# MP-Gadget/shenqi

Measured on AMD Instinct MI355X. Metric: particle-steps/sec (grav+PM+SPH) at 256^3; rms force error vs ref, higher is better.
Workload: dtype f64

## Files before the change

### include/shenqi_hip.h

```cpp
#ifndef SHENQI_HIP_H
#define SHENQI_HIP_H

#include <stddef.h>
#include <stdint.h>

#ifdef __cplusplus
extern "C" {
#endif

#define SHQ_OK 0
#define SHQ_ERR_INVALID 1
#define SHQ_ERR_DEVICE 2
#define SHQ_ERR_NOMEM 3
#define SHQ_ERR_STATE 4
#define SHQ_ERR_NOCONV 5

#define SHQ_NGRAVTAB 512
#define SHQ_NMAXCHILD 8
#define SHQ_NODELISTLENGTH 4
#define SHQ_TIMEBINS 46

typedef struct shq_context shq_context;


// ... 350 lines not shown
    double Imom[3][3];
    double Jmom[3];
    double MaxDens;
    int64_t first_member;
} shq_fof_group;
int shq_fof(shq_context *ctx, const shq_fof_params *params, const uint64_t *ids, uint64_t *minid_by_particle, int32_t *grnr_by_particle,
            int64_t *ngroups);
int shq_fof_groups_download(shq_context *ctx, shq_fof_group *groups, int64_t capacity);
int shq_fof_group_sums(shq_context *ctx, const double *values_by_particle, int ncol, double *sums_by_group);
int shq_fof_seed_select(shq_context *ctx, double MinFoFMassForNewSeed, double MinMStarForNewSeed, int32_t *d_seed_index, int64_t capacity, int64_t *nseeds);
int shq_fof_members(shq_context *ctx, int32_t *members, int64_t capacity, int64_t *nmembers);

typedef struct shq_bh_dyn_view {
    void *base;
    size_t elsize;
    int64_t numslots;
    size_t off_mintimebin, off_timebindynfric, off_jumptominpot;
    size_t off_dfaccel, off_df_surroundingvel, off_dragaccel;
    size_t off_minpotpos, off_minpotvel;
} shq_bh_dyn_view;
int shq_bh_dynamics_upload(shq_context *ctx, const shq_part_view *parts, const shq_bh_dyn_view *bh);
int shq_bh_dynamics_download(shq_context *ctx, const shq_part_view *parts, const shq_bh_dyn_view *bh);
int shq_set_bh_reposition(shq_context *ctx, int enabled);
int shq_kick_bh(shq_context *ctx, const double gravkick[SHQ_TIMEBINS + 1], const int32_t *active, int64_t nactive);
int shq_grav_short_run(shq_context *ctx, const shq_grav_params *params, const int32_t *active,
                       int64_t nactive, int update_potential, int walk_mode);
int shq_grav_short_run_range(shq_context *ctx, const shq_grav_params *params, int64_t first, int64_t count,
                             int update_potential, int walk_mode);
int shq_set_walk_stats(shq_context *ctx, int level);
int shq_set_walk_launch(shq_context *ctx, int persist, int leaf_ring);
int shq_set_walk_sparse(shq_context *ctx, int enable);
int shq_walk_pair_lean(shq_context *ctx);
int shq_set_walk_overlap(shq_context *ctx, int mode);
int shq_walk_pair_status(shq_context *ctx, int64_t *recovered_launches, int64_t *stack_high_water, int64_t *last_mopped_tasks);
int shq_set_walk_debug(shq_context *ctx, int pair_spin_max, int pair_stack_cap);
int shq_set_tree_debug(shq_context *ctx, int64_t initial_node_cap);
int shq_tree_build_attempts(shq_context *ctx, int *attempts);
int shq_direct_force_sample(shq_context *ctx, const double *sample_pos, int64_t ns, int64_t nsrc, double BoxSize, double G, double h,
                            int repeat, double *accel);
int shq_grav_short_download(shq_context *ctx, double (*accel)[3], double *potential,
                            int64_t *ninteractions, shq_walk_stats *stats);
typedef struct shq_grav_query {
    double Pos[3];
    int32_t NodeList[4];
    double OldAcc;
} shq_grav_query;
typedef struct shq_grav_result {
    double Acc[3];
    double Potential;
} shq_grav_result;
int shq_grav_short_secondary(shq_context *ctx, const shq_grav_params *params, const shq_grav_query *queries, int64_t nq,
                             shq_grav_result *results, int64_t *ninteractions, int update_potential);
typedef struct shq_data_index {
    int32_t Task;
    int32_t Index;
    int32_t NodeList[4];
} shq_data_index;
int shq_toptree_upload(shq_context *ctx, const shq_tree_view *tree, const shq_topleaf *topleaves, int ntopleaves);
int shq_grav_toptree_exports(shq_context *ctx, const shq_grav_params *params, const int32_t *active, int64_t nactive,
                             int32_t *exportcounts, shq_data_index *table, int64_t capacity, int64_t *nexport);
int shq_ngb_toptree_exports(shq_context *ctx, int symmetric, double BoxSize, const int32_t *active, int64_t nactive,
                            int32_t *exportcounts, shq_data_index *table, int64_t capacity, int64_t *nexport);
int shq_grav_toptree_exports_resident(shq_context *ctx, const shq_grav_params *params, const int32_t *active, int64_t nactive,
                                      int active_on_device, int ntask, int64_t *nexport, int64_t *task_counts);
int shq_grav_export_pack(shq_context *ctx, shq_grav_query *d_queries, int32_t *d_place);
int shq_grav_reduce_export_results(shq_context *ctx, const int32_t *place, const shq_grav_result *results, int64_t n,
// ... 904 lines not shown
```

### shenqi_amd/capi.py

```python
import ctypes as C
import os

import numpy as np

_HERE = os.path.dirname(os.path.abspath(__file__))
LIBDIR = os.environ.get("SHQ_LIBDIR") or os.path.join(_HERE, "lib")
DATADIR = os.path.join(_HERE, "data")

NGRAVTAB = 512
NMAXCHILD = 8
NOFIELD = C.c_size_t(-1).value

WALK_EXACT = 0
WALK_GROUP = 1
WALK_AUTO = 2
WALK_TREE_ORDER = 0x100
WALK_DEFER_POSTPROCESS = 0x200


class ShqError(RuntimeError):
    """Non-zero status from the library (the shim's endrun() equivalent)."""


def _load(name):
# ... 378 lines not shown
TOPLEAF_DTYPE = np.dtype([("Task", "<i4"), ("topnode", "<i4"), ("treenode", "<i4")])
DATA_INDEX_DTYPE = np.dtype([("Task", "<i4"), ("Index", "<i4"), ("NodeList", "<i4", 4)])
hip.shq_grav_reduce_export_results.argtypes = [_vp, _vp, _vp, C.c_int64, C.c_int]
hip.shq_grav_reduce_export_results.restype = C.c_int
hip.shq_grav_postprocess.argtypes = [_vp, C.POINTER(GravParams), _vp, C.c_int64, C.c_int]
hip.shq_grav_postprocess.restype = C.c_int
hip.shq_toptree_upload.argtypes = [_vp, C.POINTER(TreeView), _vp, C.c_int]
hip.shq_toptree_upload.restype = C.c_int
hip.shq_grav_toptree_exports.argtypes = [_vp, C.POINTER(GravParams), _vp, C.c_int64, _vp, _vp, C.c_int64, C.POINTER(C.c_int64)]
hip.shq_grav_toptree_exports.restype = C.c_int
hip.shq_ngb_toptree_exports.argtypes = [_vp, C.c_int, C.c_double, _vp, C.c_int64, _vp, _vp, C.c_int64, C.POINTER(C.c_int64)]
hip.shq_ngb_toptree_exports.restype = C.c_int
hip.shq_grav_toptree_exports_resident.argtypes = [_vp, C.POINTER(GravParams), _vp, C.c_int64, C.c_int, C.c_int, C.POINTER(C.c_int64), _vp]
hip.shq_grav_toptree_exports_resident.restype = C.c_int
hip.shq_grav_export_pack.argtypes = [_vp, _vp, _vp]
hip.shq_grav_export_pack.restype = C.c_int
GAS_NCOL = 28
hip.shq_gas_set_device.argtypes = [_vp, _vp, C.c_int64, C.c_int64]
hip.shq_gas_get_device.argtypes = [_vp, _vp, C.c_int64, C.c_int]
hip.shq_density_resident.argtypes = [_vp, C.POINTER(DensityParams), C.POINTER(SphStats)]
hip.shq_hydro_resident.argtypes = [_vp, C.POINTER(HydroParams), C.POINTER(SphStats)]
for _f in ("shq_gas_set_device", "shq_gas_get_device", "shq_density_resident", "shq_hydro_resident"):
    getattr(hip, _f).restype = C.c_int
hip.shq_set_walk_stats.argtypes = [_vp, C.c_int]
hip.shq_set_walk_stats.restype = C.c_int
hip.shq_set_walk_launch.argtypes = [_vp, C.c_int, C.c_int]
hip.shq_set_walk_launch.restype = C.c_int
hip.shq_set_walk_sparse.argtypes = [_vp, C.c_int]
hip.shq_set_walk_sparse.restype = C.c_int
hip.shq_walk_pair_lean.argtypes = [_vp]
hip.shq_walk_pair_lean.restype = C.c_int
hip.shq_set_walk_overlap.argtypes = [_vp, C.c_int]
hip.shq_set_walk_overlap.restype = C.c_int
hip.shq_pm_set_fft_transposed.argtypes = [_vp, C.c_int]
hip.shq_pm_set_fft_transposed.restype = C.c_int
hip.shq_walk_pair_status.argtypes = [_vp, C.POINTER(C.c_int64), C.POINTER(C.c_int64), C.POINTER(C.c_int64)]
hip.shq_walk_pair_status.restype = C.c_int
hip.shq_set_walk_debug.argtypes = [_vp, C.c_int, C.c_int]
hip.shq_set_walk_debug.restype = C.c_int
hip.shq_set_tree_debug.argtypes = [_vp, C.c_int64]
hip.shq_set_tree_debug.restype = C.c_int
hip.shq_tree_build_attempts.argtypes = [_vp, C.POINTER(C.c_int)]
hip.shq_tree_build_attempts.restype = C.c_int
hip.shq_direct_force_sample.argtypes = [_vp, _vp, C.c_int64, C.c_int64, C.c_double, C.c_double, C.c_double, C.c_int, _vp]
hip.shq_direct_force_sample.restype = C.c_int
hip.shq_exchange_plan.argtypes = [_vp, C.POINTER(ExchangeLayout), _vp, C.c_int64, _vp, C.c_int, C.c_int, C.c_int64, C.POINTER(C.c_int64), C.POINTER(C.c_int64), _vp]
hip.shq_exchange_pack.argtypes = [_vp, C.POINTER(ExchangeLayout), _vp, _vp, C.c_int64, _vp, C.c_int, _vp, _vp]
hip.shq_exchange_unpack.argtypes = [_vp, C.POINTER(ExchangeLayout), _vp, C.c_int64, _vp, _vp, _vp, C.c_int]
hip.shq_slots_gc.argtypes = [_vp, C.POINTER(ExchangeLayout), _vp, C.POINTER(C.c_int64), C.c_int64, _vp, _vp, _vp]
hip.shq_slots_gc_sorted.argtypes = [_vp, C.POINTER(ExchangeLayout), _vp, C.POINTER(C.c_int64), C.c_int64, _vp, _vp, _vp]
hip.shq_slots_split_particles.argtypes = [_vp, C.POINTER(ExchangeLayout), C.POINTER(SpawnLayout), _vp, C.POINTER(C.c_int64), C.c_int64, _vp, _vp, C.c_int64, _vp]
hip.shq_slots_convert.argtypes = [_vp, C.POINTER(ExchangeLayout), _vp, C.c_int64, C.c_int64, _vp, _vp, _vp, _vp, C.c_int64, C.c_int]
hip.shq_make_particle_stars.argtypes = [_vp, C.POINTER(ExchangeLayout), C.POINTER(StarSpawnLayout), _vp, C.c_int64, C.c_int64, _vp, _vp, _vp, _vp, _vp, C.c_int64, C.c_double]
hip.shq_blackhole_make_seeds.argtypes = [_vp, C.POINTER(ExchangeLayout), C.POINTER(BhSeedLayout), _vp, C.c_int64, C.c_int64, _vp, _vp, _vp, _vp, _vp, C.c_int64,
                                         C.c_double, C.c_double]
hip.shq_bh_accretion.argtypes = [_vp, C.POINTER(TreeView), C.POINTER(PartView), C.POINTER(SphView), C.POINTER(BhSlotView), _vp, _vp, C.c_int64, C.POINTER(KickFactors),
                                 C.POINTER(BhParams), C.c_int64, _vp, C.c_int64, C.POINTER(BhWork)]
hip.shq_bh_feedback.argtypes = [_vp, C.POINTER(TreeView), C.POINTER(PartView), C.POINTER(SphView), C.POINTER(BhSlotView), _vp, _vp, C.c_int64, C.POINTER(KickFactors),
                                C.POINTER(BhParams), C.c_int64, _vp, C.c_int64, _vp, C.POINTER(BhWork), C.POINTER(C.c_int64), C.POINTER(C.c_int64)]
hip.shq_bh_accretion.restype = hip.shq_bh_feedback.restype = C.c_int
hip.shq_winds_and_feedback.argtypes = [_vp, C.POINTER(TreeView), C.POINTER(PartView), C.POINTER(SphView), C.POINTER(StarView), _vp, _vp, C.c_int64, C.POINTER(WindParams),
                                       _vp, C.c_int64, _vp, _vp, C.c_int64, C.POINTER(C.c_int64), C.POINTER(C.c_int64)]
hip.shq_winds_and_feedback.restype = C.c_int
hip.shq_winds_candidates.argtypes = [_vp, C.POINTER(TreeView), C.POINTER(PartView), C.POINTER(SphView), C.POINTER(StarView), _vp, _vp, C.c_int64, C.POINTER(WindParams),
                                     _vp, C.c_int64, _vp, _vp, C.c_int64, C.POINTER(C.c_int64)]
hip.shq_winds_apply.argtypes = [_vp, C.POINTER(PartView), C.POINTER(SphView), _vp, _vp, C.c_int64, C.POINTER(WindParams), _vp, C.c_int64, C.POINTER(C.c_int64)]
# ... 862 lines not shown
```

### shenqi_amd/csrc/capi.hip

```cpp
#include "common.hpp"
#include <stdarg.h>
#include <string.h>
#include <stdlib.h>
#include <math.h>
#include <thread>
#include <atomic>
#include <algorithm>

static thread_local char g_err[1024] = "";

void shq_set_error(const char *fmt, ...)
{
    va_list ap;
    va_start(ap, fmt);
    vsnprintf(g_err, sizeof(g_err), fmt, ap);
    va_end(ap);
}

extern "C" const char *shq_last_error(void) { return g_err; }
extern "C" const char *shq_version(void) { return "shenqi_hip 0.1 (gfx950)"; }

namespace {

template <typename F> void parallel_for(int64_t n, F f)
// ... 124 lines not shown
       hipEventCreateWithFlags(&ctx->ev_pair_join, hipEventDisableTiming) != hipSuccess) {
        shq_set_error("creating the pair kernel's stream failed");
        delete ctx;
        return SHQ_ERR_DEVICE;
    }
    if(const char *v = getenv("SHQ_WALK_FREE_CUS")) {
        const int k = atoi(v);
        if(k > 0 && k <= 16) {
            uint32_t mask_walk[8];
            for(int w = 0; w < 8; w++)
                mask_walk[w] = ~0u;
            for(int a = 0; a < 8; a++)
                for(int c = 0; c < k; c++) {
                    const int bit = 32 * a + ((a + c / 4) % 8) + 8 * (c % 4);
                    mask_walk[bit >> 5] &= ~(1u << (bit & 31));
                }
            if(hipExtStreamCreateWithCUMask(&ctx->stream_walk, 8, mask_walk) != hipSuccess ||
               hipEventCreateWithFlags(&ctx->ev_walk_in, hipEventDisableTiming) != hipSuccess ||
               hipEventCreateWithFlags(&ctx->ev_walk_out, hipEventDisableTiming) != hipSuccess) {
                shq_set_error("creating the CU-masked walk stream failed");
                delete ctx;
                return SHQ_ERR_DEVICE;
            }
        }
    }
    if(const char *v = getenv("SHQ_PM_OVERLAP"))
        ctx->pm_overlap = atoi(v) != 0;
    if(const char *v = getenv("SHQ_PM_SCRUB"))
        ctx->pm_scrub = atoi(v) != 0;
    if(const char *v = getenv("SHQ_WALK_SPARSE"))
        ctx->walk_sparse = atoi(v);
    if(const char *v = getenv("SHQ_WALK_OVERLAP"))
        ctx->walk_overlap = atoi(v);
    if(const char *v = getenv("SHQ_TREE_TARGETS_REFRESH"))
        ctx->tree_targets_refresh = atoi(v) > 0 ? atoi(v) : 1;
    if(const char *v = getenv("SHQ_FFT_TRANSPOSED"))
        ctx->fft_transposed = atoi(v) != 0;
    if(const char *v = getenv("SHQ_TREEPM_FUSE"))
        ctx->treepm_fuse = atoi(v) != 0;
    if(const char *v = getenv("SHQ_WALK_VARIANT"))
        ctx->walk_variant = atoi(v);
    if(const char *v = getenv("SHQ_WALK_STATS_GUARD"))
        ctx->stats_guard = atoi(v);
    if(const char *v = getenv("SHQ_WALK_PADDING"))
        ctx->allow_padding = atoi(v) != 0;
    if(const char *v = getenv("SHQ_WALK_STATS"))
        ctx->walk_stats = atoi(v);
    if(const char *v = getenv("SHQ_XCD_K"))
        ctx->xcd_k = atoi(v);
    if(const char *v = getenv("SHQ_WALK_PERSIST"))
        ctx->walk_persist = atoi(v);
    if(const char *v = getenv("SHQ_WALK_RING"))
        ctx->walk_ring = atoi(v);
    {
        int ncu = 0;
        if(hipDeviceGetAttribute(&ncu, hipDeviceAttributeMultiprocessorCount, device) == hipSuccess && ncu > 0)
            ctx->num_cus = ncu;
    }
    *out = ctx;
    return SHQ_OK;
}

extern "C" void shq_shutdown(shq_context *ctx)
{
    if(!ctx)
        return;
// ... 65 lines not shown
        (void) hipStreamDestroy(ctx->stream);
    if(ctx->stream_walk)
        (void) hipStreamDestroy(ctx->stream_walk);
    if(ctx->stream_pm)
        (void) hipStreamDestroy(ctx->stream_pm);
    if(ctx->stream_pair)
        (void) hipStreamDestroy(ctx->stream_pair);
    if(ctx->ev_pair_fork)
        (void) hipEventDestroy(ctx->ev_pair_fork);
    if(ctx->ev_pair_join)
        (void) hipEventDestroy(ctx->ev_pair_join);
    for(int i = 0; i < 4; i++)
        if(ctx->ev_sph[i])
            (void) hipEventDestroy(ctx->ev_sph[i]);
    if(ctx->ev_pm_ready)
        (void) hipEventDestroy(ctx->ev_pm_ready);
    if(ctx->ev_pm_done)
        (void) hipEventDestroy(ctx->ev_pm_done);
    delete ctx;
}

extern "C" int shq_set_walk_sparse(shq_context *ctx, int enable)
{
    SHQ_CHECK(ctx, SHQ_ERR_INVALID, "null context");
    ctx->walk_sparse = enable == 2 ? 2 : enable != 0;
    return SHQ_OK;
}

extern "C" int shq_set_walk_overlap(shq_context *ctx, int mode)
{
    SHQ_CHECK(ctx, SHQ_ERR_INVALID, "null context");
    SHQ_CHECK(mode >= 0 && mode <= 2, SHQ_ERR_INVALID, "walk overlap mode %d", mode);
    ctx->walk_overlap = mode;
    return SHQ_OK;
}

extern "C" int shq_walk_pair_lean(shq_context *ctx)
{
    SHQ_CHECK(ctx, SHQ_ERR_INVALID, "null context");
    if(!ctx->node_lean_checked || !ctx->node_lean_bad.ptr)
        return 0;
    SHQ_HIP(hipSetDevice(ctx->device));
    int bad = 1;
    SHQ_HIP(hipMemcpyAsync(&bad, ctx->node_lean_bad.ptr, sizeof(int), hipMemcpyDeviceToHost, ctx->stream));
    SHQ_HIP(hipStreamSynchronize(ctx->stream));
    return bad == 0 ? 1 : 0;
}

extern "C" int shq_set_walk_launch(shq_context *ctx, int persist, int leaf_ring)
{
    SHQ_CHECK(ctx && persist >= 0 && persist <= 2 && (leaf_ring == 0 || leaf_ring == 1), SHQ_ERR_INVALID, "walk launch: persist 0..2, leaf_ring 0 or 1");
    ctx->walk_persist = persist;
    ctx->walk_ring = leaf_ring;
    return SHQ_OK;
}

extern "C" int shq_set_walk_stats(shq_context *ctx, int level)
{
    SHQ_CHECK(ctx && level >= 0 && level <= 2, SHQ_ERR_INVALID, "walk stats level must be 0, 1 or 2");
    ctx->walk_stats = level;
    return SHQ_OK;
}

int shq_join_pm(shq_context *ctx)
{
    if(ctx->pm_pending) {
// ... 1172 lines not shown
```

### shenqi_amd/csrc/common.hpp

```cpp
#ifndef SHQ_COMMON_HPP
#define SHQ_COMMON_HPP

#include <hip/hip_runtime.h>
#include <hipfft/hipfft.h>
#include <stdint.h>
#include <stdio.h>
#include <string>
#include <vector>
#include "../../include/shenqi_hip.h"
#include "yields_math.hpp"
#include "cooling_math.hpp"

void shq_set_error(const char *fmt, ...);

#define SHQ_HIP(call)                                                                          \
    do {                                                                                       \
        hipError_t e_ = (call);                                                                \
        if(e_ != hipSuccess) {                                                                 \
            shq_set_error("%s:%d: %s failed: %s", __FILE__, __LINE__, #call, hipGetErrorString(e_)); \
            return (e_ == hipErrorOutOfMemory) ? SHQ_ERR_NOMEM : SHQ_ERR_DEVICE;               \
        }                                                                                      \
    } while(0)

#define SHQ_CHECK(cond, code, ...)                                                             \
// ... 389 lines not shown
    bool pm_measure_power = false;
    bool have_power = false;
    int ps_nbins = 0, ps_bintab_n = 0;
    DevBuf<double> ps_sums;
    DevBuf<int32_t> ps_bintab;
    bool pm_spec_pending = false;
    shq_pm_params pm_spec_params = {};
    int pm_spec_route = 0;
    DevBuf<double> pm_fac;
    bool pm_fac_set = false;
    DevBuf<double> pm_fac_one;
    int pm_typemask = -1;
    DevBuf<double> slab_fac;
    bool ps_slab = false;
    bool have_types = false;

    shq_walk_stats last_stats = {};
    int walk_variant = 3;
    int walk_stats = 0;
    int walk_persist = 1;
    int walk_ring = 1;
    int num_cus = 256;
    DevBuf<unsigned int> walk_tasks;
    DevBuf<int4> sp_items, sp_stack;
    DevBuf<int32_t> sp_count;
    DevBuf<int> sp_flags;
    PinBuf<int> sp_host;
    int sp_stack_cap = 0;
    unsigned sp_spin_max = 0;
    int walk_sparse = 1;
    DevBuf<int> node_lean_bad;
    bool node_lean_checked = false;
    int walk_overlap = 1;
    bool sp_check_pending = false;
    int xcd_k = 32;
    float last_walk_ms = 0;
    int last_walk_mode = 0;

    PinBuf<char> stage;

    bool uvbg_keep = false;
    int uvbg_n = 0;
    std::vector<float> uvbg_j21, uvbg_xhi;
    double uvbg_ms[4] = {0, 0, 0, 0};
    shq_heiii_stats heiii_stats = {};
    double lens_ms[4] = {0, 0, 0, 0};
    DevBuf<double> zel_spec;
    bool zel_have = false;
    int zel_n = 0, zel_seed = 0, zel_unitary = 0, zel_invert = 0;
    int64_t zel_chunk = 0;
    double zel_ms[4] = {0, 0, 0, 0};
    double glass_ms[4] = {0, 0, 0, 0};
    double thermal_ms[3] = {0, 0, 0};
    bool yld_have = false;
    YieldDesc yld_desc = {};
    std::vector<double> yld_host;
    DevBuf<double> yld_tab, yld_time;
    int64_t yld_time_n = 0;
    double yld_loga0 = 0, yld_dloga = 0, yld_amin = 0, yld_amax = 0;
    DevBuf<double> yld_in, yld_out;
    DevBuf<int32_t> yld_i32;
    DevBuf<uint8_t> yld_mark;
    double yld_ms[2] = {0, 0};
    bool cool_have = false;
    CoolPar cool_par = {};
    double cool_fbar = 0;
// ... 242 lines not shown
```

### shenqi_amd/csrc/grav_walk.hip

```cpp
#include "common.hpp"
#include "pm_readout.hpp"
#include <utility>
#include <stdlib.h>

namespace {

struct WalkArgs {
    const NodeG *nodeG;
    const double4 *posm;
    const double4 *posm_leaf;
    const double *oldacc;
    const int32_t *targets;
    const int32_t *qstart;
    double *acc;
    double *pot;
    int32_t *nint;
    GravStatsDev *stats;
    long long ntargets;
    int root;
    double Box, invBox, halfBox;
    double rcut, rcut2;
    double h, h2, h_inv, h3_inv;
    double inv_celldx;
    double errtol, bh2;
// ... 144 lines not shown
#define SHQ_SPARSE_LANES 8
#endif
#ifndef SHQ_SPARSE_CAP
#define SHQ_SPARSE_CAP 96
#endif
#define SHQ_SPARSE_STACK 4096
#define SHQ_SPARSE_SPIN (1u << 22)
#ifndef SHQ_PAIR_DEPTH2
#define SHQ_PAIR_DEPTH2 1
#endif
enum SpFlag {
    SP_OVERFLOW = 0,
    SP_GAVEUP = 1,
    SP_MOPPED = 2,
    SP_HIGHWATER = 3,
    SP_STICKY_ERROR = 8,
    SP_STICKY_RECOVERED = 9,
    SP_STICKY_HIGHWATER = 10,
    SP_TASK_COUNTER = 16
};
#define SP_TASK_DONE (-2)
#ifndef SHQ_PAIR_WAVES
#define SHQ_PAIR_WAVES 8
#define SHQ_PAIR_WG_PER_CU 2
#define SHQ_PAIR_EU 4
#endif

template <bool POT>
__device__ __forceinline__ void leaf_ring_drain(const double4 *__restrict__ tab, const double4 *ring, unsigned &mymask, double px, double py,
                                                double pz, const WalkArgs &a, double &ax, double &ay, double &az, double &pot,
                                                const unsigned long long wrapm)
{
    asm volatile("s_waitcnt vmcnt(0)" ::: "memory");
    while(shq_ballot(mymask != 0u) != 0ull) {
        if(mymask != 0u) {
            const int b = __builtin_ctz(mymask);
            mymask &= mymask - 1u;
            const double4 q = ring[b];
            leaf_particle<POT>(tab, q, px, py, pz, a, ax, ay, az, pot, wrapm);
        }
    }
}

template <bool POT, bool PREFETCH, int LEAFB, int STATS, bool BH, bool GHOSTS = false, bool PERSIST = false, bool RING = false, bool READOUT = false,
          bool SPARSE = false>
__global__ __launch_bounds__(512) __attribute__((amdgpu_num_sgpr(96), amdgpu_num_vgpr(64))) void grav_walk_exact_kernel(const WalkArgs a)
{
    extern __shared__ double4 ring_all[];
    double4 *const ring = ring_all + (threadIdx.x >> 6) * SHQ_LEAF_RING;
    __shared__ double4 tab[SHQ_NGRAVTAB];
    for(int i = threadIdx.x; i < SHQ_NGRAVTAB; i += blockDim.x) {
        const int j = (i + 1 < SHQ_NGRAVTAB) ? i + 1 : i;
        const double f0 = a.tab_f[i], f1 = a.tab_f[j], p0 = a.tab_p[i], p1 = a.tab_p[j];
        tab[i] = i + 1 < SHQ_NGRAVTAB ? make_double4(f0, f1 - f0, p0, p1 - p0) : make_double4(0, 0, 0, 0);
    }
    __syncthreads();

    typedef const SHQ_CONSTANT_AS NodeG *NodeGK;
    typedef const SHQ_CONSTANT_AS double4 *Double4K;
    const NodeGK nodeG = (NodeGK) (size_t) a.nodeG;
    const Double4K posm_leaf = (Double4K) (size_t) a.posm_leaf;
    const int lane = threadIdx.x & 63;
    int region = blockIdx.x & 7, tried = 0;
    long long wave = PERSIST ? (long long) walk_next_task(walk_cold_args(), region, tried)
                             : (long long) xcd_block(blockIdx.x, gridDim.x, a.xcdK) * (blockDim.x >> 6) + (threadIdx.x >> 6);
    while(wave >= 0) {
    const long long t = wave * 64 + lane;
    long long pi = 0;
    double px = 0, py = 0, pz = 0, aold = 0;
    bool valid;
    {
        const WalkArgs c = PERSIST ? *walk_cold_args() : a;
        valid = t < c.ntargets;
        if(valid) {
            pi = c.targets ? (long long) c.targets[t] : t;
            valid = pi >= 0;
        }
        if(valid) {
// ... 32 lines not shown
                if(u0 + k < c.scrub_n16) {
                    unsigned z = 0;
                    asm volatile("" : "+v"(z));
                    c.scrub[u0 + k] = make_uint4(z, z, z, z);
                }
        }
    }
    double ax = 0, ay = 0, az = 0, pot = 0;
    int nint = 0;
    int sp_n = 0;
    unsigned ringmask = 0;
    int ringfill = 0;
    unsigned long long ringwrap = 0;
    unsigned int node_int_wave = 0;
    int mynext = valid ? a.root : -2;
    int cur = a.root;
    int wrapnode = -1;
    int seg1 = -1, seg2 = -1, seg3 = -1, myend = -1;
    if(GHOSTS) {
        mynext = -2;
        if(valid) {
            const int4 st = *reinterpret_cast<const int4 *>(a.qstart + 4 * t);
            mynext = st.x >= 0 ? st.x : -2;
            seg1 = st.y; seg2 = st.z; seg3 = st.w;
            if(mynext >= 0)
                myend = a.nodeG[mynext].sibling;
        }
    }
    unsigned int visited = 0, wave_applies = 0, wave_node_applies = 0;
    unsigned int hv[8] = {}, hn[8] = {}, hl[8] = {};
    unsigned int lonely8 = 0, lonely16 = 0;

    do {
        NodeG nd = nodeG[cur];
        int wl_hi = __double2hiint(nd.wraplim);
        asm volatile("" : "+s"(wl_hi));
        nd.wraplim = __hiloint2double(wl_hi, __double2loint(nd.wraplim));
        if(STATS)
            visited++;
        const bool act = (mynext == cur);
        if(STATS == 2)
            hv[(__popcll(shq_ballot(mynext == cur)) - 1) >> 3 & 7]++;

        double dx = nd.cofm[0] - px, dy = nd.cofm[1] - py, dz = nd.cofm[2] - pz;
        double ux = nd.center[0] - px, uy = nd.center[1] - py, uz = nd.center[2] - pz;
        double cmax = fmax(fmax(fabs(ux), fabs(uy)), fabs(uz));
        const unsigned long long actm = shq_ballot(mynext == cur);
        if(wl_hi >= 0) {
            asm volatile("" ::: "memory");
            const unsigned long long wrapm = shq_ballot(cmax >= nd.wraplim) & actm;
            if(wrapm != 0ull) {
                wrapnode = cur;
                dx = wrapd(dx, a.Box, a.invBox);
                dy = wrapd(dy, a.Box, a.invBox);
                dz = wrapd(dz, a.Box, a.invBox);
                ux = wrapd(ux, a.Box, a.invBox);
                uy = wrapd(uy, a.Box, a.invBox);
                uz = wrapd(uz, a.Box, a.invBox);
                cmax = fmax(fmax(fabs(ux), fabs(uy)), fabs(uz));
            }
        }
        const double r2 = fma(dz, dz, fma(dy, dy, dx * dx));
        const unsigned long long keepm = actm & ~(shq_ballot(r2 > nd.rcut2) & shq_ballot(cmax > nd.rcuthl));
        const unsigned long long openm = (BH ? 0ull : shq_ballot(nd.mlen2 > r2 * r2 * aold)) | shq_ballot(r2 < nd.bhlim) |
                                         shq_ballot(cmax < nd.inside);
        const unsigned long long acceptm = keepm & ~openm, doopenm = keepm & openm;
        const bool accept = __builtin_amdgcn_inverse_ballot_w64(acceptm), doopen = __builtin_amdgcn_inverse_ballot_w64(doopenm);

        {
            if(STATS && acceptm != 0ull) {
                wave_applies++;
                wave_node_applies++;
                node_int_wave += (unsigned int) __popcll(acceptm);
            }
            if(STATS == 2 && acceptm != 0ull) {
                const int pc = __popcll(acceptm);
                hn[(pc - 1) >> 3 & 7]++;
                if(accept && pc <= 8)
                    lonely8++;
                if(accept && pc <= 16)
                    lonely16++;
            }
            if(accept) {
                apply_accn<POT, false>(tab, dx, dy, dz, r2, nd.mass, a, ax, ay, az, pot);
                nint++;
            }
        }
        if(nd.type == SHQ_PARTICLE_NODE_TYPE) {
            asm volatile("" ::: "memory");
            if(RING && doopenm != 0ull) {
                const int cnt = nd.count;
                if(ringfill + cnt > SHQ_LEAF_RING) {
                    leaf_ring_drain<POT>(tab, ring, ringmask, px, py, pz, a, ax, ay, az, pot, ringwrap);
                    ringfill = 0;
                    ringwrap = 0;
                }
                if(lane < 2 * cnt)
                    __builtin_amdgcn_global_load_lds(reinterpret_cast<const double2 *>(a.posm_leaf + nd.child) + lane,
                                                     (__attribute__((address_space(3))) void *) (ring + ringfill), 16, 0, 0);
                if(doopen) {
                    ringmask |= ((1u << cnt) - 1u) << ringfill;
                    nint += cnt;
                }
                ringfill += cnt;
                if(wrapnode == cur)
                    ringwrap = 1ull;
            }
            if(!RING && doopenm != 0ull) {
                const unsigned long long wrapm = wrapnode == cur ? 1ull : 0ull;
                const Double4K lp = posm_leaf + nd.child;
                const int cnt = nd.count;
                if(STATS)
                    wave_applies += cnt;
                if(STATS == 2) {
                    const int pc = __popcll(doopenm);
                    hl[(pc - 1) >> 3 & 7] += cnt;
                    if(doopen && pc <= 8)
                        lonely8 += cnt;
                    if(doopen && pc <= 16)
                        lonely16 += cnt;
                }
#pragma unroll
                for(int b = 0; b < SHQ_NMAXCHILD; b += LEAFB) {
                    if(b < cnt) {
                        double4 q[LEAFB];
#pragma unroll
                        for(int k = 0; k < LEAFB; k++)
                            q[k] = lp[b + k];
                        if(doopen) {
#pragma unroll
                            for(int k = 0; k < LEAFB; k++)
                                if(b + k < cnt)
                                    leaf_particle<POT>(tab, q[k], px, py, pz, a, ax, ay, az, pot, wrapm);
                        }
                    }
                }
                if(doopen)
                    nint += cnt;
            }
            }
        unsigned long long downm = 0ull;
        int next = nd.sibling;
        if(nd.type == SHQ_NODE_NODE_TYPE) {
            asm volatile("" ::: "memory");
            if(doopenm != 0ull) {
                asm volatile("" ::: "memory");
                downm = doopenm;
                next = nd.child;
                if(SPARSE) {
                    int pc;
                    asm("s_bcnt1_i32_b64 %[pc], %[m]" : [pc] "=s"(pc) : [m] "s"(doopenm) : "scc");
                    if(((pc - (SHQ_SPARSE_LANES + 1)) & (sp_n - SHQ_SPARSE_CAP)) < 0) {
                        if(lane == 0) {
                            unsigned long long *const it = reinterpret_cast<unsigned long long *>(walk_cold_args()->sp_items + (wave * SHQ_SPARSE_CAP + sp_n));
                            agent_store(it, ((unsigned long long) (unsigned) nd.sibling << 32) | (unsigned) nd.child);
                            agent_store(it + 1, doopenm);
                        }
                        sp_n++;
                        downm = 0ull;
                        next = nd.sibling;
                    }
                }
            }
            if(GHOSTS) {
                if(shq_ballot(mynext > cur && (nd.sibling < 0 || mynext < nd.sibling)) != 0ull)
                    next = nd.child;
            }
        }
        {
            const unsigned long long staym = actm & ~downm;
            asm volatile("s_mov_b64 exec, %[m1]\n\t"
                         "v_mov_b32 %[dst], %[sib]\n\t"
                         "s_mov_b64 exec, %[m2]\n\t"
                         "v_mov_b32 %[dst], %[chd]\n\t"
                         "s_mov_b64 exec, -1"
                         : [dst] "+v"(mynext)
                         : [m1] "s"(staym), [m2] "s"(downm), [sib] "s"(nd.sibling), [chd] "s"(nd.child));
        }
        if(GHOSTS && act && mynext == myend) {
            mynext = seg1 >= 0 ? seg1 : -2;
            seg1 = seg2;
            seg2 = seg3;
            seg3 = -1;
            myend = mynext >= 0 ? a.nodeG[mynext].sibling : -1;
        }
        cur = __builtin_amdgcn_readfirstlane(next);
    } while(cur >= 0);

    if(RING)
        leaf_ring_drain<POT>(tab, ring, ringmask, px, py, pz, a, ax, ay, az, pot, ringwrap);
    {
    const WalkArgs c = PERSIST ? *walk_cold_args() : a;
    if(valid) {
        if(SPARSE) {
            agent_store(&c.acc[3 * pi + 0], ax);
            agent_store(&c.acc[3 * pi + 1], ay);
            agent_store(&c.acc[3 * pi + 2], az);
            if(POT)
                agent_store(&c.pot[pi], pot);
            agent_store(&c.nint[pi], (int32_t) nint);
        } else {
            c.acc[3 * pi + 0] = ax;
            c.acc[3 * pi + 1] = ay;
            c.acc[3 * pi + 2] = az;
            if(POT)
                c.pot[pi] = pot;
            c.nint[pi] = nint;
        }
    }
    if(SPARSE) {
        asm volatile("s_waitcnt vmcnt(0)" ::: "memory");
        if(lane == 0)
            agent_store(&c.sp_count[wave], (int32_t) sp_n);
    }
    long long mn = valid ? (long long) nint : __double_as_longlong(sconst(__longlong_as_double(0x7fffffffffffll))), mx = valid ? nint : 0, sm = valid ? nint : 0;
    for(int off = 32; off > 0; off >>= 1) {
        long long o1 = __shfl_xor(mn, off), o2 = __shfl_xor(mx, off), o3 = __shfl_xor(sm, off);
        mn = o1 < mn ? o1 : mn;
        mx = o2 > mx ? o2 : mx;
        sm += o3;
    }
    unsigned int l8s = lonely8, l8m = lonely8, l16s = lonely16, l16m = lonely16;
    if(STATS == 2)
// ... 391 lines not shown
        double M = Box;
        for(int k = 0; k < 3; k++)
            M = fmin(M, fmin(g[i].center[k] - hl, Box - (g[i].center[k] + hl)));
        const double wl = fmax(0.5 * Box - hl, 0.0);
        g[i].wraplim = (len > 0 && wl > 0 && M >= rcut + 1.5 * len) ? -wl : wl;
        if(lean_bad && i < n - 1) {
            const double rootlen = Box * 1.001;
            const int k = lean_level(rootlen, len);
            const LeanProducts lp = lean_products(g[i].mass, len, rcut, Box);
            const bool ok = len > 0 && k >= 0 && k < 32 && ldexp(rootlen, -k) == len && lp.rcuthl == g[i].rcuthl &&
                            lp.mlen2 == g[i].mlen2 && lp.inside == g[i].inside && lp.wraplim == wl;
            if(!ok)
                *lean_bad = 1;
        }
    }
}

__global__ void stats_init_kernel(GravStatsDev *s)
{
    s->ninteractions = 0;
    s->nvisited = 0;
    s->nwave_applies = 0;
    s->nwave_node_applies = 0;
    s->nnode_interactions = 0;
    s->min_int = 0x7fffffffffffll;
    s->max_int = 0;
    for(int b = 0; b < 8; b++)
        s->hist_visit[b] = s->hist_node[b] = s->hist_leaf[b] = 0;
    for(int b = 0; b < 4; b++)
        s->lonely[b] = 0;
}

template <bool POT, bool PREFETCH, int LEAFB, bool BH>
void launch_variant_bh(int stats, bool persist, dim3 grid, dim3 block, hipStream_t stream, const WalkArgs &a, size_t dyn_lds = 0)
{
    constexpr bool RO = !PREFETCH && LEAFB == 2 && !BH;
    if(a.pm_mesh && a.sp_items && RO && !stats && persist && block.x == 512)
        grav_walk_exact_kernel<POT, PREFETCH, LEAFB, 0, BH, false, RO, RO, RO, RO><<<grid, block, dyn_lds, stream>>>(a);
    else if(a.sp_items && RO && !stats && persist && block.x == 512)
        grav_walk_exact_kernel<POT, PREFETCH, LEAFB, 0, BH, false, RO, RO, false, RO><<<grid, block, dyn_lds, stream>>>(a);
    else if(a.pm_mesh && RO && !stats && persist && block.x == 512)
        grav_walk_exact_kernel<POT, PREFETCH, LEAFB, 0, BH, false, RO, RO, RO><<<grid, block, dyn_lds, stream>>>(a);
    else if(a.pm_mesh && RO && !stats && !persist)
        grav_walk_exact_kernel<POT, PREFETCH, LEAFB, 0, BH, false, false, false, RO><<<grid, block, 0, stream>>>(a);
    else if(stats == 2 && POT && !PREFETCH && LEAFB == 2)
        grav_walk_exact_kernel<POT, PREFETCH, LEAFB, (POT && !PREFETCH && LEAFB == 2) ? 2 : 1, BH><<<grid, block, 0, stream>>>(a);
    else if(stats)
        grav_walk_exact_kernel<POT, PREFETCH, LEAFB, 1, BH><<<grid, block, 0, stream>>>(a);
    else if(persist && !PREFETCH && LEAFB == 2 && block.x == 512)
        grav_walk_exact_kernel<POT, PREFETCH, LEAFB, 0, BH, false, (!PREFETCH && LEAFB == 2), (!PREFETCH && LEAFB == 2)><<<grid, block, dyn_lds, stream>>>(a);
    else if(persist && !PREFETCH && LEAFB == 2)
        grav_walk_exact_kernel<POT, PREFETCH, LEAFB, 0, BH, false, (!PREFETCH && LEAFB == 2)><<<grid, block, dyn_lds, stream>>>(a);
    else
        grav_walk_exact_kernel<POT, PREFETCH, LEAFB, 0, BH><<<grid, block, 0, stream>>>(a);
}

template <bool POT, bool PREFETCH, int LEAFB>
void launch_variant(int stats, bool persist, dim3 grid, dim3 block, hipStream_t stream, const WalkArgs &a, size_t dyn_lds = 0)
{
    if(a.useBH)
        launch_variant_bh<POT, PREFETCH, LEAFB, true>(stats, persist, grid, block, stream, a, dyn_lds);
    else
        launch_variant_bh<POT, PREFETCH, LEAFB, false>(stats, persist, grid, block, stream, a, dyn_lds);
}

}

void shq_launch_stats_init(shq_context *ctx) { stats_init_kernel<<<1, 1, 0, ctx->stream>>>(ctx->gstats.ptr); }

void shq_fill_node_walk_params(shq_context *ctx, const shq_grav_params *p)
{
    if((ctx->node_rcut != p->Rcut || ctx->node_bh2 != p->BHOpeningAngle2) && ctx->numnodes > 0) {
        const long long n = ctx->numnodes + 1;
        int *lean_bad = nullptr;
        if(ctx->node_lean_bad.reserve(16) == SHQ_OK && hipMemsetAsync(ctx->node_lean_bad.ptr, 0, sizeof(int) * 16, ctx->stream) == hipSuccess)
            lean_bad = ctx->node_lean_bad.ptr;
        ctx->node_lean_checked = lean_bad != nullptr;
        fill_rcuthl_kernel<<<dim3((unsigned) ((n + 255) / 256)), dim3(256), 0, ctx->stream>>>(ctx->nodeG.ptr, n, p->Rcut, p->BHOpeningAngle2, p->BoxSize, lean_bad);
        ctx->node_rcut = p->Rcut;
        ctx->node_bh2 = p->BHOpeningAngle2;
    }
}

static void fill_walk_args(shq_context *ctx, const shq_grav_params *p, WalkArgs &a)
{
    shq_fill_node_walk_params(ctx, p);
    a.nodeG = ctx->nodeG.ptr;
    a.posm = ctx->posm.ptr;
    a.posm_leaf = ctx->posm_leaf.ptr;
    a.oldacc = ctx->oldacc.ptr;
    a.targets = nullptr;
    a.qstart = nullptr;
    a.acc = ctx->acc.ptr;
    a.pot = ctx->pot.ptr;
    a.nint = ctx->nint.ptr;
    a.stats = ctx->gstats.ptr;
    a.ntargets = 0;
    a.root = ctx->root;
    a.Box = p->BoxSize;
// ... 268 lines not shown
        if(ctx->mesh_words % 2 == 0 && per <= 4096) {
            a.scrub = (uint4 *) ctx->mesh.ptr;
            a.scrub_n16 = n16;
            a.scrub_per_task = (int) per;
            scrubbed = true;
        }
    }
    if(ctx->fuse_readout) {
        SHQ_CHECK(shq_walk_can_fuse_readout(ctx, p, d_active, ntargets, first), SHQ_ERR_STATE, "fused readout requested for a launch that cannot carry it");
        a.pm_mesh = ctx->mesh.ptr;
        a.pmN = ctx->pm_nmesh;
        a.pmzp = ctx->pm_zp;
        a.pmcell = ctx->fuse_cell;
        a.pmffac = ctx->fuse_ffac;
        a.G = ctx->fuse_G;
        a.treeacc = ctx->treeacc.ptr;
        a.pflags = ctx->pflags.ptr;
        a.gravpm = ctx->gravpm.ptr;
        a.pmpot = ctx->pmpot.ptr;
        a.oldacc_out = ctx->oldacc.ptr;
        if(scrubbed && ctx->mesh_alt.reserve(ctx->mesh_words) == SHQ_OK) {
            a.scrub = (uint4 *) ctx->mesh_alt.ptr;
            swap_meshes = true;
        } else {
            a.scrub = nullptr;
            a.scrub_per_task = 0;
            scrubbed = false;
        }
    }
    const dim3 grid((unsigned) launch_blocks), block(ring ? 512 : threads);
    SHQ_HIP(hipEventRecord(ctx->ev_begin[SHQ_T_WALK], ctx->stream));
    if(live)
        SHQ_HIP(hipEventRecord(ctx->ev_pair_fork, ctx->stream));
    if(update_potential) {
        switch(variant) {
        case 0: launch_variant<true, false, 4>(stats, persist, grid, block, ctx->stream, a); break;
        case 1: launch_variant<true, false, 2>(stats, persist, grid, block, ctx->stream, a); break;
        case 2: launch_variant<true, false, 4>(stats, persist, grid, block, ctx->stream, a); break;
        default: launch_variant<true, false, 2>(stats, persist, grid, block, ctx->stream, a, dyn_lds); break;
        }
    } else {
        switch(variant) {
        case 0: launch_variant<false, false, 4>(stats, persist, grid, block, ctx->stream, a); break;
        case 1: launch_variant<false, false, 2>(stats, persist, grid, block, ctx->stream, a); break;
        case 2: launch_variant<false, false, 4>(stats, persist, grid, block, ctx->stream, a); break;
        default: launch_variant<false, false, 2>(stats, persist, grid, block, ctx->stream, a, dyn_lds); break;
        }
    }
    SHQ_HIP(hipGetLastError());
    if(sparse) {
        hipStream_t ps = live ? ctx->stream_pair : ctx->stream;
        if(live)
            SHQ_HIP(hipStreamWaitEvent(ps, ctx->ev_pair_fork, 0));
        const dim3 pg((unsigned) pair_blocks);
        if(live) {
            if(update_potential)
                grav_pair_kernel_live<true><<<pg, dim3(256), 0, ps>>>(a);
            else
                grav_pair_kernel_live<false><<<pg, dim3(256), 0, ps>>>(a);
        } else if(update_potential)
            grav_pair_kernel<true><<<pg, dim3(64 * SHQ_PAIR_WAVES), 0, ps>>>(a);
        else
            grav_pair_kernel<false><<<pg, dim3(64 * SHQ_PAIR_WAVES), 0, ps>>>(a);
        SHQ_HIP(hipGetLastError());
        if(live) {
            SHQ_HIP(hipEventRecord(ctx->ev_pair_join, ps));
            SHQ_HIP(hipStreamWaitEvent(ctx->stream, ctx->ev_pair_join, 0));
            WalkArgs m = a;
            m.sp_live = 0;
            m.sp_mop = 1;
            const dim3 mg((unsigned) mop_blocks);
            if(update_potential)
                grav_pair_kernel<true><<<mg, dim3(64 * SHQ_PAIR_WAVES), 0, ctx->stream>>>(m);
            else
                grav_pair_kernel<false><<<mg, dim3(64 * SHQ_PAIR_WAVES), 0, ctx->stream>>>(m);
            SHQ_HIP(hipGetLastError());
        }
        SHQ_HIP(hipMemcpyAsync(ctx->sp_host.ptr, ctx->sp_flags.ptr + SP_STICKY_ERROR, sizeof(int) * 8, hipMemcpyDeviceToHost, ctx->stream));
        ctx->sp_check_pending = true;
    }
    SHQ_HIP(hipEventRecord(ctx->ev_end[SHQ_T_WALK], ctx->stream));
    if(swap_meshes) {
// ... 114 lines not shown
```

Baseline: 428.3 million.

## Fetch tree node records with 32-bit-offset scalar loads in the walk kernel

Adds an ADDR32 variant of the exact tree walk that loads each 128-byte node record with explicit scalar s_load instructions, using a 32-bit byte offset from the node pool base. This variant is used when the node count fits and the sparse persistent path is selected. It also replaces branchy per-lane updates of the ring mask, interaction count and next-node pointer with exec-masked inline assembly. These changes are meant to cut address arithmetic and divergence overhead in the hot walk loop. In exchange it relies on a fixed NodeG layout and hand-written exec manipulation, and it changes the GHOSTS ballot condition.

```diff
diff --git a/include/shenqi_hip.h b/include/shenqi_hip.h
--- a/include/shenqi_hip.h
+++ b/include/shenqi_hip.h
@@ -406,6 +406,9 @@
 int shq_set_walk_sparse(shq_context *ctx, int enable);
 int shq_walk_pair_lean(shq_context *ctx);
 int shq_set_walk_overlap(shq_context *ctx, int mode);
+int shq_set_walk_addr(shq_context *ctx, int mode);
+int shq_walk_last_addr(shq_context *ctx, int *mode);
+int shq_walk_addr32_fits(int64_t numnodes);
 int shq_walk_pair_status(shq_context *ctx, int64_t *recovered_launches, int64_t *stack_high_water, int64_t *last_mopped_tasks);
 int shq_set_walk_debug(shq_context *ctx, int pair_spin_max, int pair_stack_cap);
 int shq_set_tree_debug(shq_context *ctx, int64_t initial_node_cap);
diff --git a/shenqi_amd/capi.py b/shenqi_amd/capi.py
--- a/shenqi_amd/capi.py
+++ b/shenqi_amd/capi.py
@@ -434,6 +434,12 @@
 hip.shq_walk_pair_lean.restype = C.c_int
 hip.shq_set_walk_overlap.argtypes = [_vp, C.c_int]
 hip.shq_set_walk_overlap.restype = C.c_int
+hip.shq_set_walk_addr.argtypes = [_vp, C.c_int]
+hip.shq_set_walk_addr.restype = C.c_int
+hip.shq_walk_last_addr.argtypes = [_vp, C.POINTER(C.c_int)]
+hip.shq_walk_last_addr.restype = C.c_int
+hip.shq_walk_addr32_fits.argtypes = [C.c_int64]
+hip.shq_walk_addr32_fits.restype = C.c_int
 hip.shq_pm_set_fft_transposed.argtypes = [_vp, C.c_int]
 hip.shq_pm_set_fft_transposed.restype = C.c_int
 hip.shq_walk_pair_status.argtypes = [_vp, C.POINTER(C.c_int64), C.POINTER(C.c_int64), C.POINTER(C.c_int64)]
diff --git a/shenqi_amd/csrc/capi.hip b/shenqi_amd/csrc/capi.hip
--- a/shenqi_amd/csrc/capi.hip
+++ b/shenqi_amd/csrc/capi.hip
@@ -180,6 +180,8 @@
         ctx->walk_sparse = atoi(v);
     if(const char *v = getenv("SHQ_WALK_OVERLAP"))
         ctx->walk_overlap = atoi(v);
+    if(const char *v = getenv("SHQ_WALK_ADDR"))
+        ctx->walk_addr = atoi(v) != 0;
     if(const char *v = getenv("SHQ_TREE_TARGETS_REFRESH"))
         ctx->tree_targets_refresh = atoi(v) > 0 ? atoi(v) : 1;
     if(const char *v = getenv("SHQ_FFT_TRANSPOSED"))
@@ -311,6 +313,21 @@
     SHQ_CHECK(ctx, SHQ_ERR_INVALID, "null context");
     SHQ_CHECK(mode >= 0 && mode <= 2, SHQ_ERR_INVALID, "walk overlap mode %d", mode);
     ctx->walk_overlap = mode;
+    return SHQ_OK;
+}
+
+extern "C" int shq_set_walk_addr(shq_context *ctx, int mode)
+{
+    SHQ_CHECK(ctx, SHQ_ERR_INVALID, "null context");
+    SHQ_CHECK(mode == 0 || mode == 1, SHQ_ERR_INVALID, "walk addr mode %d", mode);
+    ctx->walk_addr = mode;
+    return SHQ_OK;
+}
+
+extern "C" int shq_walk_last_addr(shq_context *ctx, int *mode)
+{
+    SHQ_CHECK(ctx && mode, SHQ_ERR_INVALID, "null argument");
+    *mode = ctx->last_walk_addr32 ? 1 : 0;
     return SHQ_OK;
 }
 
diff --git a/shenqi_amd/csrc/common.hpp b/shenqi_amd/csrc/common.hpp
--- a/shenqi_amd/csrc/common.hpp
+++ b/shenqi_amd/csrc/common.hpp
@@ -445,6 +445,8 @@
     DevBuf<int> node_lean_bad;
     bool node_lean_checked = false;
     int walk_overlap = 1;
+    int walk_addr = 1;
+    bool last_walk_addr32 = false;
     bool sp_check_pending = false;
     int xcd_k = 32;
     float last_walk_ms = 0;
diff --git a/shenqi_amd/csrc/grav_walk.hip b/shenqi_amd/csrc/grav_walk.hip
--- a/shenqi_amd/csrc/grav_walk.hip
+++ b/shenqi_amd/csrc/grav_walk.hip
@@ -200,8 +200,9 @@
                                                 const unsigned long long wrapm)
 {
     asm volatile("s_waitcnt vmcnt(0)" ::: "memory");
-    while(shq_ballot(mymask != 0u) != 0ull) {
-        if(mymask != 0u) {
+    unsigned long long popm;
+    while((popm = shq_ballot(mymask != 0u)) != 0ull) {
+        if(__builtin_amdgcn_inverse_ballot_w64(popm)) {
             const int b = __builtin_ctz(mymask);
             mymask &= mymask - 1u;
             const double4 q = ring[b];
@@ -210,8 +211,14 @@
     }
 }
 
+typedef unsigned int walk_u32x4 __attribute__((ext_vector_type(4)));
+typedef unsigned int walk_u32x8 __attribute__((ext_vector_type(8)));
+typedef unsigned int walk_u32x16 __attribute__((ext_vector_type(16)));
+__device__ __forceinline__ double walk_f64(unsigned lo, unsigned hi) { return __hiloint2double((int) hi, (int) lo); }
+static_assert(offsetof(NodeG, sibling) == 0x40 && offsetof(NodeG, bhlim) == 0x50 && offsetof(NodeG, wraplim) == 0x70, "the ADDR32 fetch names the record's pieces by offset");
+
 template <bool POT, bool PREFETCH, int LEAFB, int STATS, bool BH, bool GHOSTS = false, bool PERSIST = false, bool RING = false, bool READOUT = false,
-          bool SPARSE = false>
+          bool SPARSE = false, bool ADDR32 = false>
 __global__ __launch_bounds__(512) __attribute__((amdgpu_num_sgpr(96), amdgpu_num_vgpr(64))) void grav_walk_exact_kernel(const WalkArgs a)
 {
     extern __shared__ double4 ring_all[];
@@ -310,7 +317,39 @@
     unsigned int lonely8 = 0, lonely16 = 0;
 
     do {
-        NodeG nd = nodeG[cur];
+        NodeG nd;
+        if constexpr(ADDR32) {
+            walk_u32x16 q0;
+            walk_u32x4 q1, q3;
+            walk_u32x8 q2;
+            const unsigned recoff = (unsigned) cur << 7;
+            asm volatile("s_load_dwordx4 %[q3], %[pool], %[off] offset:0x70\n\t"
+                         "s_load_dwordx16 %[q0], %[pool], %[off] offset:0x0\n\t"
+                         "s_load_dwordx4 %[q1], %[pool], %[off] offset:0x40\n\t"
+                         "s_load_dwordx8 %[q2], %[pool], %[off] offset:0x50\n\t"
+                         "s_waitcnt lgkmcnt(0)"
+                         : [q0] "=&s"(q0), [q1] "=&s"(q1), [q2] "=&s"(q2), [q3] "=&s"(q3)
+                         : [pool] "s"((unsigned long long) (size_t) a.nodeG), [off] "s"(recoff));
+            nd.cofm[0] = walk_f64(q0[0], q0[1]);
+            nd.cofm[1] = walk_f64(q0[2], q0[3]);
+            nd.cofm[2] = walk_f64(q0[4], q0[5]);
+            nd.mass = walk_f64(q0[6], q0[7]);
+            nd.center[0] = walk_f64(q0[8], q0[9]);
+            nd.center[1] = walk_f64(q0[10], q0[11]);
+            nd.center[2] = walk_f64(q0[12], q0[13]);
+            nd.len = walk_f64(q0[14], q0[15]);
+            nd.sibling = (int) q1[0];
+            nd.child = (int) q1[1];
+            nd.type = (int) q1[2];
+            nd.count = (int) q1[3];
+            nd.bhlim = walk_f64(q2[0], q2[1]);
+            nd.mlen2 = walk_f64(q2[2], q2[3]);
+            nd.inside = walk_f64(q2[4], q2[5]);
+            nd.rcut2 = walk_f64(q2[6], q2[7]);
+            nd.wraplim = walk_f64(q3[0], q3[1]);
+            nd.rcuthl = walk_f64(q3[2], q3[3]);
+        } else
+            nd = nodeG[cur];
         int wl_hi = __double2hiint(nd.wraplim);
         asm volatile("" : "+s"(wl_hi));
         nd.wraplim = __hiloint2double(wl_hi, __double2loint(nd.wraplim));
@@ -376,9 +415,14 @@
                 if(lane < 2 * cnt)
                     __builtin_amdgcn_global_load_lds(reinterpret_cast<const double2 *>(a.posm_leaf + nd.child) + lane,
                                                      (__attribute__((address_space(3))) void *) (ring + ringfill), 16, 0, 0);
-                if(doopen) {
-                    ringmask |= ((1u << cnt) - 1u) << ringfill;
-                    nint += cnt;
+                {
+                    const unsigned slots = ((1u << cnt) - 1u) << ringfill;
+                    asm volatile("s_mov_b64 exec, %[m]\n\t"
+                                 "v_or_b32 %[rm], %[slots], %[rm]\n\t"
+                                 "v_add_u32 %[ni], %[cnt], %[ni]\n\t"
+                                 "s_mov_b64 exec, -1"
+                                 : [rm] "+v"(ringmask), [ni] "+v"(nint)
+                                 : [m] "s"(doopenm), [slots] "s"(slots), [cnt] "s"(cnt));
                 }
                 ringfill += cnt;
                 if(wrapnode == cur)
@@ -413,17 +457,24 @@
                         }
                     }
                 }
-                if(doopen)
-                    nint += cnt;
-            }
-            }
-        unsigned long long downm = 0ull;
+                asm volatile("s_mov_b64 exec, %[m]\n\t"
+                             "v_add_u32 %[ni], %[cnt], %[ni]\n\t"
+                             "s_mov_b64 exec, -1"
+                             : [ni] "+v"(nint)
+                             : [m] "s"(doopenm), [cnt] "s"(cnt));
+            }
+            }
         int next = nd.sibling;
+        asm volatile("s_mov_b64 exec, %[m]\n\t"
+                     "v_mov_b32 %[dst], %[sib]\n\t"
+                     "s_mov_b64 exec, -1"
+                     : [dst] "+v"(mynext)
+                     : [m] "s"(actm), [sib] "s"(nd.sibling));
         if(nd.type == SHQ_NODE_NODE_TYPE) {
             asm volatile("" ::: "memory");
             if(doopenm != 0ull) {
                 asm volatile("" ::: "memory");
-                downm = doopenm;
+                unsigned long long downm = doopenm;
                 next = nd.child;
                 if(SPARSE) {
                     int pc;
@@ -439,21 +490,16 @@
                         next = nd.sibling;
                     }
                 }
+                asm volatile("s_mov_b64 exec, %[m]\n\t"
+                             "v_mov_b32 %[dst], %[chd]\n\t"
+                             "s_mov_b64 exec, -1"
+                             : [dst] "+v"(mynext)
+                             : [m] "s"(downm), [chd] "s"(nd.child));
             }
             if(GHOSTS) {
-                if(shq_ballot(mynext > cur && (nd.sibling < 0 || mynext < nd.sibling)) != 0ull)
+                if(shq_ballot(!act && mynext > cur && (nd.sibling < 0 || mynext < nd.sibling)) != 0ull)
                     next = nd.child;
             }
-        }
-        {
-            const unsigned long long staym = actm & ~downm;
-            asm volatile("s_mov_b64 exec, %[m1]\n\t"
-                         "v_mov_b32 %[dst], %[sib]\n\t"
-                         "s_mov_b64 exec, %[m2]\n\t"
-                         "v_mov_b32 %[dst], %[chd]\n\t"
-                         "s_mov_b64 exec, -1"
-                         : [dst] "+v"(mynext)
-                         : [m1] "s"(staym), [m2] "s"(downm), [sib] "s"(nd.sibling), [chd] "s"(nd.child));
         }
         if(GHOSTS && act && mynext == myend) {
             mynext = seg1 >= 0 ? seg1 : -2;
@@ -465,8 +511,9 @@
         cur = __builtin_amdgcn_readfirstlane(next);
     } while(cur >= 0);
 
-    if(RING)
+    if(RING) {
         leaf_ring_drain<POT>(tab, ring, ringmask, px, py, pz, a, ax, ay, az, pot, ringwrap);
+    }
     {
     const WalkArgs c = PERSIST ? *walk_cold_args() : a;
     if(valid) {
@@ -924,12 +971,15 @@
 }
 
 template <bool POT, bool PREFETCH, int LEAFB, bool BH>
-void launch_variant_bh(int stats, bool persist, dim3 grid, dim3 block, hipStream_t stream, const WalkArgs &a, size_t dyn_lds = 0)
+bool launch_variant_bh(int stats, bool persist, dim3 grid, dim3 block, hipStream_t stream, const WalkArgs &a, size_t dyn_lds = 0, bool addr32 = false)
 {
     constexpr bool RO = !PREFETCH && LEAFB == 2 && !BH;
     if(a.pm_mesh && a.sp_items && RO && !stats && persist && block.x == 512)
         grav_walk_exact_kernel<POT, PREFETCH, LEAFB, 0, BH, false, RO, RO, RO, RO><<<grid, block, dyn_lds, stream>>>(a);
-    else if(a.sp_items && RO && !stats && persist && block.x == 512)
+    else if(a.sp_items && RO && !stats && persist && block.x == 512 && addr32) {
+        grav_walk_exact_kernel<POT, PREFETCH, LEAFB, 0, BH, false, RO, RO, false, RO, RO><<<grid, block, dyn_lds, stream>>>(a);
+        return true;
+    } else if(a.sp_items && RO && !stats && persist && block.x == 512)
         grav_walk_exact_kernel<POT, PREFETCH, LEAFB, 0, BH, false, RO, RO, false, RO><<<grid, block, dyn_lds, stream>>>(a);
     else if(a.pm_mesh && RO && !stats && persist && block.x == 512)
         grav_walk_exact_kernel<POT, PREFETCH, LEAFB, 0, BH, false, RO, RO, RO><<<grid, block, dyn_lds, stream>>>(a);
@@ -945,18 +995,20 @@
         grav_walk_exact_kernel<POT, PREFETCH, LEAFB, 0, BH, false, (!PREFETCH && LEAFB == 2)><<<grid, block, dyn_lds, stream>>>(a);
     else
         grav_walk_exact_kernel<POT, PREFETCH, LEAFB, 0, BH><<<grid, block, 0, stream>>>(a);
+    return false;
 }
 
 template <bool POT, bool PREFETCH, int LEAFB>
-void launch_variant(int stats, bool persist, dim3 grid, dim3 block, hipStream_t stream, const WalkArgs &a, size_t dyn_lds = 0)
+bool launch_variant(int stats, bool persist, dim3 grid, dim3 block, hipStream_t stream, const WalkArgs &a, size_t dyn_lds = 0, bool addr32 = false)
 {
     if(a.useBH)
-        launch_variant_bh<POT, PREFETCH, LEAFB, true>(stats, persist, grid, block, stream, a, dyn_lds);
-    else
-        launch_variant_bh<POT, PREFETCH, LEAFB, false>(stats, persist, grid, block, stream, a, dyn_lds);
-}
-
-}
+        return launch_variant_bh<POT, PREFETCH, LEAFB, true>(stats, persist, grid, block, stream, a, dyn_lds, addr32);
+    return launch_variant_bh<POT, PREFETCH, LEAFB, false>(stats, persist, grid, block, stream, a, dyn_lds, addr32);
+}
+
+}
+
+extern "C" int shq_walk_addr32_fits(int64_t numnodes) { return (numnodes >= 0 && numnodes + 1 <= ((int64_t) 1 << 25)) ? 1 : 0; }
 
 void shq_launch_stats_init(shq_context *ctx) { stats_init_kernel<<<1, 1, 0, ctx->stream>>>(ctx->gstats.ptr); }
 
@@ -1291,22 +1343,25 @@
     SHQ_HIP(hipEventRecord(ctx->ev_begin[SHQ_T_WALK], ctx->stream));
     if(live)
         SHQ_HIP(hipEventRecord(ctx->ev_pair_fork, ctx->stream));
+    const bool addr32 = ctx->walk_addr != 0 && shq_walk_addr32_fits(ctx->numnodes) != 0;
+    bool used32 = false;
     if(update_potential) {
         switch(variant) {
         case 0: launch_variant<true, false, 4>(stats, persist, grid, block, ctx->stream, a); break;
         case 1: launch_variant<true, false, 2>(stats, persist, grid, block, ctx->stream, a); break;
         case 2: launch_variant<true, false, 4>(stats, persist, grid, block, ctx->stream, a); break;
-        default: launch_variant<true, false, 2>(stats, persist, grid, block, ctx->stream, a, dyn_lds); break;
+        default: used32 = launch_variant<true, false, 2>(stats, persist, grid, block, ctx->stream, a, dyn_lds, addr32); break;
         }
     } else {
         switch(variant) {
         case 0: launch_variant<false, false, 4>(stats, persist, grid, block, ctx->stream, a); break;
         case 1: launch_variant<false, false, 2>(stats, persist, grid, block, ctx->stream, a); break;
         case 2: launch_variant<false, false, 4>(stats, persist, grid, block, ctx->stream, a); break;
-        default: launch_variant<false, false, 2>(stats, persist, grid, block, ctx->stream, a, dyn_lds); break;
+        default: used32 = launch_variant<false, false, 2>(stats, persist, grid, block, ctx->stream, a, dyn_lds, addr32); break;
         }
     }
     SHQ_HIP(hipGetLastError());
+    ctx->last_walk_addr32 = used32;
     if(sparse) {
         hipStream_t ps = live ? ctx->stream_pair : ctx->stream;
         if(live)
```

Result: faster. 435.2 million, median of 6 (+1.6%).
